# sara-nl/2D-VQ-AE-2

Measured on AMD Instinct MI355X. Metric: patches/sec (VQAE.forward: encoder -> VQ -> decoder), higher is better.
Workload: dtype f32; 1 GPU; BASELINE configs[1] (cfg B): batch 256/GPU of 256x256x3 fp32 -> 32x32 codes, K=256, D=128, full forward; global_batch=256, parallelism=patch-sharded x1

## Files before the change

### 2d-vq-ae-2_amd/csrc/conv_wino43.hip

```cpp
#include "kernels.h"
#include "mfma.h"

namespace {

using namespace vqae;

struct W43K {
    const float* __restrict__ t1;
    const float* __restrict__ U;
    const float* __restrict__ w3;
    const float* __restrict__ w1n;
    float* xio;
    float* y2;
    const float* __restrict__ Us;
    const float* __restrict__ w3s;
    const float* __restrict__ w1ns;
    int H, M;
    float act_a, act_b, t_scale, t_b4, n_b1a, n_b1b, n_b2a, n_b2b;
};

template <int C_, bool WIDE_ = false> struct W43Cfg {
    static constexpr int C = C_;
    static constexpr bool WIDE = WIDE_;
    static constexpr int BANDS = WIDE ? 2 : 1;
    static constexpr int ROWS = 8 * BANDS;
    static constexpr int W = C >= 128 ? 32 : 64;
    static constexpr int NT = (C == 256 || WIDE) ? 512 : 256;
    static constexpr int NWV = NT / 64;
    static constexpr int NS = C / 32;
    static constexpr int TG = NWV / NS;
    static constexpr int TILES = 16 * TG;
    static constexpr int TC = W / 4;
    static constexpr int PXH = 4 * W * BANDS;
    static constexpr int C4 = C / 4;
    static constexpr int RP = NT / C4;
    static constexpr int LDT = C + 4;
    static constexpr int KG = C / 16;
    static constexpr int KS = C / 8;
    static constexpr int NI = 2;
    static constexpr int WN = C / (32 * NI);
    static constexpr int MI = PXH / ((NWV / WN) * 32);
    static constexpr int V_BYTES = 6 * TILES * LDT * 4, T_BYTES = PXH * LDT * 4;
    static constexpr int LDS_BYTES = V_BYTES > T_BYTES ? V_BYTES : T_BYTES;
    static constexpr int LDVB = 3 * C + 8, KC = C / 32, KS2 = C / 16;
    static constexpr int VS_BYTES = 6 * TILES * LDVB * 2;
    static constexpr int LDS_SPLIT = VS_BYTES > T_BYTES ? VS_BYTES : T_BYTES;
    static_assert(TILES == 2 * TC * BANDS && RP == TC * BANDS && PXH / RP == 16 && MI * NI == 4, "geometry");
    static_assert(!WIDE || C == 128, "the wide form serves C = 128");
};
constexpr int EARLY = 1;
constexpr int RD = 4;
constexpr int NRES0 = 4;
constexpr int RT = 3;

__device__ __forceinline__ void split3(const f32x4& v, bf16x4 (&h)[3]) {
    h[0] = __builtin_convertvector(v, bf16x4);
    const f32x4 r1 = v - __builtin_convertvector(h[0], f32x4);
    h[1] = __builtin_convertvector(r1, bf16x4);
    const f32x4 r2 = r1 - __builtin_convertvector(h[1], f32x4);
    h[2] = __builtin_convertvector(r2, bf16x4);
}
__device__ __forceinline__ bf16x8 as_bf8(const f32x4& v) { return __builtin_bit_cast(bf16x8, v); }

__device__ __forceinline__ f32x4 fma4(const f32x4& a, float s, const f32x4& c) {
    return __builtin_elementwise_fma(a, f32x4{s, s, s, s}, c);
}

__device__ __forceinline__ f32x4 ldg(const float* sbase, unsigned voff_bytes) {
    return *reinterpret_cast<const f32x4*>(reinterpret_cast<const char*>(sbase) + voff_bytes);
}

template <int N> struct IC { static constexpr int value = N; };

constexpr int tail_row(int r) { return 8 * (r >> 2) + 4 * ((r >> 1) & 1) + (r & 1); }

template <int C, int TAIL, bool SPLIT, bool WIDE = false>
__global__ __launch_bounds__((W43Cfg<C, WIDE>::NT), (W43Cfg<C, WIDE>::NT == 512 ? 1 : 2))
void wino43_trunk_kernel(const W43K p) {
    using K = W43Cfg<C, WIDE>;
    static_assert(!WIDE || SPLIT, "the wide form is a split form");
    constexpr int W = K::W, LDT = K::LDT, KG = K::KG, KS = K::KS, TILES = K::TILES, TC = K::TC, NS = K::NS, C4 = K::C4, RP = K::RP;
    constexpr int MI = K::MI, NI = K::NI, WN = K::WN;
    constexpr int LDVB = K::LDVB, KC = K::KC, KS2 = K::KS2;
    extern __shared__ __attribute__((aligned(16))) float lds[];
    const int tid = threadIdx.x;
    const int lane = tid & 63;
    const int wave = __builtin_amdgcn_readfirstlane(tid >> 6);
    const int li = lane & 15, q = lane >> 4;
    const int ns = WIDE ? wave >> 1 : wave % NS, tg = WIDE ? 0 : wave / NS;

    int tile_m;
    {
        const int nwg = gridDim.x, bid = blockIdx.x;
        const int qq = nwg >> 3, r = nwg & 7, xcd = bid & 7;
        tile_m = (xcd < r ? xcd * (qq + 1) : r * (qq + 1) + (xcd - r) * qq) + (bid >> 3);
    }
    const int tpi = p.H / K::ROWS;
    const int img = tile_m / tpi;
    const int row0 = K::ROWS * (tile_m - img * tpi);
    const float* const xim = p.t1 + (int64_t)img * p.H * W * C;

    const int cg = tid % C4, tj = tid / C4;
    const int xcg = WIDE ? 8 * (wave & 3) + (lane & 7) : cg, tjc = WIDE ? lane >> 3 : tj, band = WIDE ? wave >> 2 : 0;
    constexpr int NCOL = WIDE ? 4 : 6, NB = NCOL / 2;
    unsigned coff[NCOL];
    int roff[2][6];
#pragma unroll
    for (int j = 0; j < NCOL; ++j) coff[j] = (unsigned)((((4 * tjc - 1 + j) & (W - 1)) * C + 4 * xcg) * 4);
#pragma unroll
    for (int s = 0; s < 2; ++s)
#pragma unroll
        for (int i = 0; i < 6; ++i) {
            int r = row0 + 8 * band + 4 * s - 1 + i;
            r = r < 0 ? r + p.H : (r >= p.H ? r - p.H : r);
            roff[s][i] = r * W * C;
        }

    f32x4 d[2][4][2];
    f32x4 w[6];
    auto issue = [&](auto kind_c, int k) __attribute__((always_inline)) {
        constexpr int KIND = decltype(kind_c)::value;
        const int s = k / NB, cp = k % NB, bf = k & 1;
#pragma unroll
        for (int i = 0; i < (KIND == 1 ? 4 : 3); ++i) {
            const int row = KIND == 0 ? 2 * i : (KIND == 5 ? 2 * i + 1 : i + 1);
#pragma unroll
            for (int jj = 0; jj < 2; ++jj) d[bf][i][jj] = ldg(xim + roff[s][row], coff[2 * cp + jj]);
        }
    };
    auto combine = [&](auto kind_c, int k, float c1, float c2, float c3) __attribute__((always_inline)) {
        constexpr int KIND = decltype(kind_c)::value;
        const int cp = k % NB, bf = k & 1;
#pragma unroll
        for (int jj = 0; jj < 2; ++jj) {
            if (KIND == 1) w[2 * cp + jj] = fma4(d[bf][0][jj], c1, fma4(d[bf][1][jj], c2, fma4(d[bf][2][jj], c3, d[bf][3][jj])));
            else w[2 * cp + jj] = fma4(d[bf][0][jj], 4.f, fma4(d[bf][1][jj], -5.f, d[bf][2][jj]));
        }
    };
    auto exchange = [&]() __attribute__((always_inline)) {
        const int nb = 4 * ((lane + 8) & 63);
#pragma unroll
        for (int jj = 0; jj < 2; ++jj)
#pragma unroll
            for (int e = 0; e < 4; ++e) {
                const float mine = w[jj][e];
                w[4 + jj][e] = __int_as_float(__builtin_amdgcn_ds_bpermute(nb, __float_as_int(mine)));
            }
    };
    auto columns = [&](int s) __attribute__((always_inline)) {
        const int slot = WIDE ? 4 * (tjc & 3) + 2 * (tjc >> 2) + s : s * TC + tjc;
        float* const dst = lds + (16 * band + slot) * LDT + 4 * xcg;
        __bf16* const dsb = reinterpret_cast<__bf16*>(lds) + (16 * band + slot) * LDVB + 4 * xcg;
        int vhi = 3 * TILES * LDVB;
        if constexpr (WIDE) asm volatile("" : "+v"(vhi));
        auto put = [&](int nu, const f32x4& v) __attribute__((always_inline)) {
            if constexpr (SPLIT) {
                bf16x4 h[3];
                split3(v, h);
#pragma unroll
                for (int pl = 0; pl < 3; ++pl) {
                    if (WIDE && nu >= 3) *reinterpret_cast<bf16x4*>(dsb + vhi + (nu - 3) * TILES * LDVB + pl * C) = h[pl];
                    else *reinterpret_cast<bf16x4*>(dsb + nu * TILES * LDVB + pl * C) = h[pl];
                }
            } else {
                *reinterpret_cast<f32x4*>(dst + nu * TILES * LDT) = v;
            }
        };
        const f32x4 t1 = fma4(w[2], -4.f, w[4]), t2 = fma4(w[1], -4.f, w[3]);
        const f32x4 t3 = w[4] - w[2], t4 = w[3] - w[1];
        put(0, fma4(w[0], 4.f, fma4(w[2], -5.f, w[4])));
        put(1, t1 + t2);
        put(2, t1 - t2);
        put(3, fma4(t4, 2.f, t3));
        put(4, fma4(t4, -2.f, t3));
        put(5, fma4(w[1], 4.f, fma4(w[3], -5.f, w[5])));
    };

    const float* const ub = p.U + ns * (KG * 512);
    const float* const ubs = p.Us + ns * (KC * 1536) + (WIDE ? 768 * (wave & 1) : 0);
    const __bf16* const vbs = reinterpret_cast<const __bf16*>(lds) + (16 * tg + li) * LDVB + 8 * q;
    const unsigned wl = 16u * lane;
    const float* const bfrag = lds + (16 * tg + li) * LDT + 4 * q;

    f32x4 Y[4][4][2];
#pragma unroll
    for (int a = 0; a < 4; ++a)
#pragma unroll
        for (int b = 0; b < 4; ++b) { Y[a][b][0] = f32x4{0.f, 0.f, 0.f, 0.f}; Y[a][b][1] = f32x4{0.f, 0.f, 0.f, 0.f}; }

    auto pass = [&](auto kind_c, auto next_c, int xi, float c1, float c2, float c3, float a1, float a2, float a3) __attribute__((always_inline)) {
        constexpr int KIND = decltype(kind_c)::value;
        constexpr int NEXT = decltype(next_c)::value;
        __builtin_amdgcn_sched_barrier(0);
#pragma unroll
        for (int j = 0; j < NCOL; ++j) asm volatile("" : "+v"(coff[j]));
        if (EARLY < 1) issue(kind_c, 0);
        if (EARLY < 2) issue(kind_c, 1);
#pragma unroll
        for (int k = 0; k < 2 * NB; ++k) {
            combine(kind_c, k, c1, c2, c3);
            if (k % NB == NB - 1) {
                if constexpr (WIDE) exchange();
                columns(k / NB);
            }
            if (k + 2 < 2 * NB) issue(kind_c, k + 2);
        }
        __builtin_amdgcn_sched_barrier(0);
        f32x4 Z[4][2];
        f32x4 acc[2][2];
        auto fold_nu = [&](int nu) __attribute__((always_inline)) {
#pragma unroll
            for (int bl = 0; bl < 2; ++bl) {
                if (nu == 0) Z[0][bl] = Z[0][bl] + acc[0][bl];
                if (nu == 2) {
                    const f32x4 sm = acc[1][bl] + acc[0][bl], df = acc[1][bl] - acc[0][bl];
                    Z[0][bl] = Z[0][bl] + sm; Z[2][bl] = Z[2][bl] + sm;
                    Z[1][bl] = Z[1][bl] + df; Z[3][bl] = Z[3][bl] + df;
                }
                if (nu == 4) {
                    const f32x4 sm = acc[1][bl] + acc[0][bl], df = acc[1][bl] - acc[0][bl];
                    Z[0][bl] = Z[0][bl] + sm; Z[2][bl] = fma4(sm, 4.f, Z[2][bl]);
                    Z[1][bl] = fma4(df, 2.f, Z[1][bl]); Z[3][bl] = fma4(df, 8.f, Z[3][bl]);
                }
                if (nu == 5) Z[3][bl] = Z[3][bl] + acc[1][bl];
            }
            if (nu == 0 || nu == 2 || nu == 4)
                asm volatile("" : "+v"(Z[0][0]), "+v"(Z[0][1]), "+v"(Z[1][0]), "+v"(Z[1][1]), "+v"(Z[2][0]), "+v"(Z[2][1]), "+v"(Z[3][0]), "+v"(Z[3][1]));
        };
        if constexpr (WIDE) {
            int64_t uoff = (int64_t)xi * 6 * (3 * C * C / 2);
            asm volatile("" : "+s"(uoff));
// ... 42 lines not shown
                    __builtin_amdgcn_sched_barrier(0);
                }
                fold_nu(nu);
            }
#undef WS
#undef VB
        } else if constexpr (SPLIT) {
            int64_t uoff = (int64_t)xi * 6 * (3 * C * C / 2);
            asm volatile("" : "+s"(uoff));
            const float* const ux = ubs + uoff;
#define WS(s, bl, pl) (((s) / KC) * (3 * C * C / 2) + 1536 * ((s) % KC) + 256 * (3 * (bl) + (pl)))
#define VB(s, pl) (*reinterpret_cast<const bf16x8*>(vbs + ((s) / KC) * TILES * LDVB + (pl) * C + 32 * ((s) % KC)))
            f32x4 w0[2][2], w1[2], w2[2];
#pragma unroll
            for (int bl = 0; bl < 2; ++bl) {
                w0[0][bl] = ldg(ux + WS(0, bl, 0), wl);
                w1[bl] = ldg(ux + WS(0, bl, 1), wl);
                w2[bl] = ldg(ux + WS(0, bl, 2), wl);
                w0[1][bl] = ldg(ux + WS(1, bl, 0), wl);
            }
            lds_barrier();
#pragma unroll
            for (int b = 0; b < 4; ++b) { Z[b][0] = f32x4{0.f, 0.f, 0.f, 0.f}; Z[b][1] = f32x4{0.f, 0.f, 0.f, 0.f}; }
            bf16x8 vb0 = VB(0, 0), vb1 = VB(0, 1), vb2 = VB(0, 2);
#pragma unroll
            for (int nu = 0; nu < 6; ++nu) {
                const int st = nu & 1;
                acc[st][0] = f32x4{0.f, 0.f, 0.f, 0.f};
                acc[st][1] = f32x4{0.f, 0.f, 0.f, 0.f};
#pragma unroll
                for (int kc = 0; kc < KC; ++kc) {
                    const int s = KC * nu + kc, sl = s & 1;
                    const bool nxt = s + 1 < 6 * KC;
#define MM(wa, vb) for (int bl = 0; bl < 2; ++bl) acc[st][bl] = __builtin_amdgcn_mfma_f32_16x16x32_bf16(as_bf8(wa[bl]), vb, acc[st][bl], 0, 0, 0)
                    MM(w1, vb1);
                    MM(w1, vb0);
                    if (nxt) for (int bl = 0; bl < 2; ++bl) w1[bl] = ldg(ux + WS(s + 1, bl, 1), wl);
                    MM(w2, vb0);
                    if (nxt) for (int bl = 0; bl < 2; ++bl) w2[bl] = ldg(ux + WS(s + 1, bl, 2), wl);
                    MM(w0[sl], vb2);
                    if (nxt) vb2 = VB(s + 1, 2);
                    MM(w0[sl], vb1);
                    if (nxt) vb1 = VB(s + 1, 1);
                    MM(w0[sl], vb0);
                    if (s + 2 < 6 * KC) for (int bl = 0; bl < 2; ++bl) w0[sl][bl] = ldg(ux + WS(s + 2, bl, 0), wl);
                    if (nxt) vb0 = VB(s + 1, 0);
#undef MM
                    __builtin_amdgcn_sched_barrier(0);
                }
                fold_nu(nu);
            }
#undef WS
#undef VB
        } else {
            int64_t uoff = (int64_t)xi * 6 * (C * C);
            asm volatile("" : "+s"(uoff));
            const float* const ux = ub + uoff;
#define WB(s) (((s) / KG) * (C * C) + 512 * ((s) % KG))
            f32x4 wq[RD][2];
#pragma unroll
            for (int s = 0; s < RD; ++s) {
                wq[s][0] = ldg(ux + WB(s), wl);
                wq[s][1] = ldg(ux + WB(s) + 256, wl);
            }
            lds_barrier();
#pragma unroll
            for (int b = 0; b < 4; ++b) { Z[b][0] = f32x4{0.f, 0.f, 0.f, 0.f}; Z[b][1] = f32x4{0.f, 0.f, 0.f, 0.f}; }
            f32x4 bq[2];
            bq[0] = *reinterpret_cast<const f32x4*>(bfrag);
#pragma unroll
            for (int nu = 0; nu < 6; ++nu) {
                const int st = nu & 1;
                acc[st][0] = f32x4{0.f, 0.f, 0.f, 0.f};
                acc[st][1] = f32x4{0.f, 0.f, 0.f, 0.f};
#pragma unroll
                for (int kg = 0; kg < KG; ++kg) {
                    const int s = KG * nu + kg;
                    if (s + 1 < 6 * KG)
                        bq[(s + 1) & 1] = *reinterpret_cast<const f32x4*>(bfrag + ((s + 1) / KG) * TILES * LDT + 16 * ((s + 1) % KG));
                    const f32x4 wa = wq[s % RD][0], wb = wq[s % RD][1];
                    if (s + RD < 6 * KG) {
                        wq[s % RD][0] = ldg(ux + WB(s + RD), wl);
                        wq[s % RD][1] = ldg(ux + WB(s + RD) + 256, wl);
                    }
#pragma unroll
                    for (int j = 0; j < 4; ++j) {
                        acc[st][0] = __builtin_amdgcn_mfma_f32_16x16x4f32(wa[j], bq[s & 1][j], acc[st][0], 0, 0, 0);
                        acc[st][1] = __builtin_amdgcn_mfma_f32_16x16x4f32(wb[j], bq[s & 1][j], acc[st][1], 0, 0, 0);
                    }
                    __builtin_amdgcn_sched_barrier(0);
                }
                fold_nu(nu);
            }
#undef WB
        }
        __builtin_amdgcn_sched_barrier(0);
        if constexpr (NEXT == 9) {
#pragma unroll
            for (int k = 0; k < EARLY; ++k)
#pragma unroll
                for (int i = 0; i < 4; ++i) {
                    const int ro = xi < 4 ? roff[0][i + 1] : roff[0][i < 3 ? 2 * i + 1 : 5];
#pragma unroll
                    for (int jj = 0; jj < 2; ++jj) d[k & 1][i][jj] = ldg(xim + ro, coff[2 * k + jj]);
                }
        } else {
// ... 111 lines not shown
                for (int mi = 0; mi < MI; ++mi) a[(ks + 1) & 1][mi] = *reinterpret_cast<const f32x4*>(a0 + mi * 32 * LDT + 8 * (ks + 1));
            }
            f32x4 bc[NI];
#pragma unroll
            for (int ni = 0; ni < NI; ++ni) bc[ni] = bt[ks % RT][ni];
            if (ks + RT < KS) {
#pragma unroll
                for (int ni = 0; ni < NI; ++ni) bt[ks % RT][ni] = ldg(b0 + ni * (KS * 256) + 256 * (ks + RT), wl);
            }
#pragma unroll
            for (int r = 0; r < 4; ++r)
#pragma unroll
                for (int mi = 0; mi < MI; ++mi)
#pragma unroll
                    for (int ni = 0; ni < NI; ++ni)
                        acc[mi][ni] = __builtin_amdgcn_mfma_f32_32x32x2f32(bc[ni][r], a[ks & 1][mi][r], acc[mi][ni], 0, 0, 0);
            __builtin_amdgcn_sched_barrier(0);
        }
    };
    auto acc_to_lds = [&]() __attribute__((always_inline)) {
#pragma unroll
        for (int ni = 0; ni < NI; ++ni)
#pragma unroll
            for (int mi = 0; mi < MI; ++mi)
#pragma unroll
                for (int g = 0; g < 4; ++g) {
                    f32x4 o;
#pragma unroll
                    for (int e = 0; e < 4; ++e) o[e] = acc[mi][ni][4 * g + e];
                    *reinterpret_cast<f32x4*>(T + (wm * MI * 32 + mi * 32 + li32) * LDT + (wn * NI + ni) * 32 + 8 * g + 4 * hh) = o;
                }
    };

#pragma unroll
    for (int hf = 0; hf < 2; ++hf) {
        int tbo = (2 * ty * W + 4 * tx) * LDT + 16 * wave + 4 * q, tro = tj0 * LDT + 4 * cg;
        if constexpr (WIDE) asm volatile("" : "+v"(tbo), "+v"(tro));
        int tbo1 = tbo + 4 * W * LDT, tro1 = tro + 8 * RP * LDT;
        if constexpr (WIDE) asm volatile("" : "+v"(tbo1), "+v"(tro1));
        auto tr = [&](int i) __attribute__((always_inline)) {
            if constexpr (WIDE) return reinterpret_cast<f32x4*>(T + (i < 8 ? tro + RP * i * LDT : tro1 + RP * (i - 8) * LDT));
            else return reinterpret_cast<f32x4*>(trow + RP * i * LDT);
        };
#pragma unroll
        for (int a2 = 0; a2 < 2; ++a2)
#pragma unroll
            for (int b = 0; b < 4; ++b)
#pragma unroll
                for (int bl = 0; bl < 2; ++bl) {
                    f32x4 o;
#pragma unroll
                    for (int e = 0; e < 4; ++e) o[e] = elu_act(Y[2 * hf + a2][b][bl][e] + p.act_a) + p.act_b;
                    if constexpr (WIDE) *reinterpret_cast<f32x4*>(T + (bl ? tbo1 : tbo) + (a2 * W + b) * LDT) = o;
                    else *reinterpret_cast<f32x4*>(T + ((2 * ty + a2) * W + 4 * tx + b) * LDT + 32 * ns + 16 * bl + 4 * q) = o;
                }
        tail_prefetch(SPLIT ? p.w3s : p.w3);
        [[maybe_unused]] float* xr[WIDE ? 1 : K::PXH / W];
        [[maybe_unused]] int64_t xu = 0;
        [[maybe_unused]] unsigned xvo = 0;
        if constexpr (WIDE) {
            xu = (((int64_t)img * p.H + row0 + 2 * hf) * W) * C;
            xvo = (unsigned)((tj0 * C + 4 * cg) * 4);
            asm volatile("" : "+v"(xvo));
        } else {
            const int64_t pixb = ((int64_t)img * p.H + row0 + 2 * hf) * W + tj0;
#pragma unroll
            for (int r = 0; r < K::PXH / W; ++r) xr[r] = p.xio + (pixb + (int64_t)(4 * (r >> 1) + (r & 1)) * W) * C + 4 * cg;
        }
        auto xp = [&](float* base, int i) __attribute__((always_inline)) {
            const int r = (RP * i) / W;
            if constexpr (WIDE) {
                int64_t ro = xu + (tail_row(r) * W + (RP * i) % W) * C;
                asm volatile("" : "+s"(ro));
                return reinterpret_cast<f32x4*>(reinterpret_cast<char*>(base + ro) + xvo);
            } else {
                return reinterpret_cast<f32x4*>(xr[r] + ((RP * i) % W) * C);
            }
        };
        f32x4 res[16];
#pragma unroll
        for (int i = 0; i < (hf == 0 ? NRES0 : 16); ++i) res[i] = __builtin_nontemporal_load(xp(p.xio, i));
        lds_barrier();
        gemm_tail(SPLIT ? p.w3s : p.w3);
        if (hf == 0) {
#pragma unroll
            for (int i = NRES0; i < 16; ++i) res[i] = __builtin_nontemporal_load(xp(p.xio, i));
        }
        if (TAIL == 2) tail_prefetch(SPLIT ? p.w1ns : p.w1n);
        lds_barrier();
        acc_to_lds();
        lds_barrier();
#pragma unroll
        for (int i = 0; i < 16; ++i) {
            f32x4 t = *tr(i);
            t = t * p.t_scale;
            t = t + p.t_b4;
            t = t + res[i];
            __builtin_nontemporal_store(t, xp(p.xio, i));
            if (TAIL == 2) {
#pragma unroll
                for (int e = 0; e < 4; ++e) t[e] = elu_act(t[e] + p.n_b1a) + p.n_b1b;
                *tr(i) = t;
            }
        }
        if constexpr (TAIL == 2) {
            lds_barrier();
// ... 60 lines not shown
        split3_f64(u[x], h);
        for (int pl = 0; pl < 3; ++pl) U[x * 3 * cc + fo + pl * 512] = h[pl];
    }
}

__global__ void split_1x1_kernel(const float* __restrict__ w, int c, __bf16* __restrict__ out) {
    const int i = blockIdx.x * blockDim.x + threadIdx.x;
    if (i >= c * c) return;
    const int n = i / c, k = i % c;
    __bf16 h[3];
    split3_f64((double)w[i], h);
    const int64_t fo = ((int64_t)(n >> 5) * (c / 16) + (k >> 4)) * 3 * 512 + (((k >> 3) & 1) * 32 + (n & 31)) * 8 + (k & 7);
    for (int pl = 0; pl < 3; ++pl) out[fo + pl * 512] = h[pl];
}

}

namespace vqae {

bool wino43_channels(int c) { return c == 256 || c == 128 || c == 64; }

bool wino43_supported(int c, int h, int w, int dtype) {
    return dtype == VQAE_DT_F32 && wino43_channels(c) && w == (c == 64 ? 64 : 32) && h >= 8 && h % 8 == 0;
}
bool wino43_enabled() { return env_int("VQAE_WINO43", 1) != 0; }

size_t wino43_weight_floats(int c) { return (size_t)36 * c * c; }

bool wino43_split_supported(int c) { return c == 128; }
size_t wino43_split_weight_bytes(int c) { return (size_t)36 * c * c * 3 * 2; }
size_t split_1x1_bytes(int c) { return (size_t)c * c * 3 * 2; }

int wino43_split_weight(const float* w_oihw_dev, int c, void* U_dev, hipStream_t stream) {
    VQAE_REQUIRE(wino43_split_supported(c), VQAE_ERR_UNSUPPORTED, "wino43_split_weight: C = %d", c);
    wino43_split_weight_kernel<<<(unsigned)ceil_div(c * c, 256), 256, 0, stream>>>(w_oihw_dev, c, (__bf16*)U_dev);
    VQAE_LAUNCH_CHECK();
    return VQAE_OK;
}

int split_1x1_weight(const float* w_packed_dev, int c, void* out_dev, hipStream_t stream) {
    VQAE_REQUIRE(wino43_split_supported(c), VQAE_ERR_UNSUPPORTED, "split_1x1_weight: C = %d", c);
    split_1x1_kernel<<<(unsigned)ceil_div(c * c, 256), 256, 0, stream>>>(w_packed_dev, c, (__bf16*)out_dev);
    VQAE_LAUNCH_CHECK();
    return VQAE_OK;
}

int wino43_transform_weight(const float* w_oihw_dev, int c, float* U_dev, hipStream_t stream) {
    VQAE_REQUIRE(wino43_channels(c), VQAE_ERR_UNSUPPORTED, "wino43_transform_weight: C = %d", c);
    wino43_weight_kernel<<<(unsigned)ceil_div(c * c, 256), 256, 0, stream>>>(w_oihw_dev, c, U_dev);
    VQAE_LAUNCH_CHECK();
    return VQAE_OK;
}

template <int C, bool SPLIT, bool WIDE = false>
static int launch_w43(W43K& k, int64_t M, bool chain, hipStream_t stream) {
    using K = W43Cfg<C, WIDE>;
    constexpr int lds = SPLIT ? K::LDS_SPLIT : K::LDS_BYTES;
    if (int rc = set_max_dynamic_lds((const void*)wino43_trunk_kernel<C, 1, SPLIT, WIDE>, lds)) return rc;
    if (int rc = set_max_dynamic_lds((const void*)wino43_trunk_kernel<C, 2, SPLIT, WIDE>, lds)) return rc;
    const unsigned grid = (unsigned)(M / (K::ROWS * K::W));
    const double flops = 2.0 * (double)M * C * (2.25 * C + C + (chain ? C : 0));
    ProfScope prof(C >= 128 ? PROF_CONV3X3_TRUNK : PROF_NONE, stream, flops);
    if (chain) wino43_trunk_kernel<C, 2, SPLIT, WIDE><<<grid, K::NT, lds, stream>>>(k);
    else wino43_trunk_kernel<C, 1, SPLIT, WIDE><<<grid, K::NT, lds, stream>>>(k);
    prof.done();
    VQAE_LAUNCH_CHECK();
    return VQAE_OK;
}

int wino43_trunk_tail(const float* t1, const float* U, const float* w3, float act_a, float act_b, float t_scale, float t_b4,
                      float* xio, const NextConv1& next, int batch, int h, int w, int c, hipStream_t stream,
                      const void* Us, const void* w3s) {
    if (batch == 0) return VQAE_OK;
    const float* w1n = (const float*)next.w1;
    float* t1_next = (float*)next.t1_next;
    VQAE_REQUIRE(t1 && U && w3 && xio && (!w1n || t1_next), VQAE_ERR_INVALID, "wino43_trunk_tail: null pointer");
    VQAE_REQUIRE(wino43_supported(c, h, w, VQAE_DT_F32), VQAE_ERR_UNSUPPORTED, "wino43_trunk_tail: C = %d, H = %d, W = %d", c, h, w);
    const int64_t M = (int64_t)batch * h * w;
    VQAE_REQUIRE(M < (1ll << 31) - 1024, VQAE_ERR_UNSUPPORTED, "wino43_trunk_tail: too many pixels");
    W43K k;
    memset(&k, 0, sizeof(k));
    k.t1 = t1; k.U = U; k.w3 = w3; k.w1n = w1n; k.xio = xio; k.y2 = t1_next;
    k.H = h; k.M = (int)M;
    k.act_a = act_a; k.act_b = act_b; k.t_scale = t_scale; k.t_b4 = t_b4;
    k.n_b1a = next.b1a; k.n_b1b = next.b1b; k.n_b2a = next.b2a; k.n_b2b = next.b2b;
    if (Us) {
        VQAE_REQUIRE(wino43_split_supported(c) && w3s && (!w1n || next.w1s), VQAE_ERR_INVALID, "wino43_trunk_tail: split form needs C = 128 and its three weights");
        k.Us = (const float*)Us; k.w3s = (const float*)w3s; k.w1ns = (const float*)next.w1s;
        if (h % 16 == 0) return launch_w43<128, true, true>(k, M, w1n != nullptr, stream);
        return launch_w43<128, true>(k, M, w1n != nullptr, stream);
    }
    switch (c) {
        case 256: return launch_w43<256, false>(k, M, w1n != nullptr, stream);
        case 128: return launch_w43<128, false>(k, M, w1n != nullptr, stream);
        default: return launch_w43<64, false>(k, M, w1n != nullptr, stream);
    }
}

}
```

### 2d-vq-ae-2_amd/csrc/handle.hip

```cpp
#include "kernels.h"

#include <algorithm>
#include <cmath>
#include <cstdlib>
#include <map>
#include <mutex>
#include <set>
#include <string>
#include <unordered_map>
#include <utility>
#include <vector>

namespace vqae {
char* last_error_buf() {
    static thread_local char buf[512] = {0};
    return buf;
}

ProfState& prof_state() {
    static ProfState p;
    return p;
}

int set_max_dynamic_lds(const void* kernel, int bytes) {
// ... 65 lines not shown
namespace {

enum { MODE_SAME = 0, MODE_DOWN = 1, MODE_UP = 2 };

struct Block : vqae::FixupScalars {
    int mode, cin, cout, br;
    float *w1, *w2, *w3, *wskip;
    float* wU43 = nullptr;
    void *wU43s = nullptr, *w1s = nullptr, *w3s = nullptr;
    float* wU = nullptr;
    float *w1f = nullptr, *w3f = nullptr;
    float *w2f = nullptr, *wskf = nullptr;
    void *w1h = nullptr, *w2h = nullptr, *w3h = nullptr, *wskh = nullptr;
    int kind = VQAE_BLOCK_FIXUP, hidden = 0;
    float *bv1 = nullptr, *bv2 = nullptr, *bv3 = nullptr;
    float *fc0w = nullptr, *fc0b = nullptr, *fc2w = nullptr, *fc2b = nullptr;
};

const float kMean255[3] = {0.7279f * 255.0f, 0.5955f * 255.0f, 0.7762f * 255.0f};
const float kInv255[3] = {1.0f / (0.2419f * 255.0f), 1.0f / (0.3083f * 255.0f), 1.0f / (0.1741f * 255.0f)};
const float kStd255[3] = {0.2419f * 255.0f, 0.3083f * 255.0f, 0.1741f * 255.0f};

}

struct vqae_handle {
    vqae_config cfg;
    int C = 0, D = 0, K = 0;
    std::vector<Block> enc, dec;
    float *stem_w = nullptr, *stem_b = nullptr, *ostem_w = nullptr, *ostem_b = nullptr;
    void *stem_wh = nullptr, *ostem_wh = nullptr;
    bool fuse_stem16 = true;
    float *embed = nullptr;
    float *pin_w = nullptr, *pin_b = nullptr, *pout_w = nullptr, *pout_b = nullptr;
    float *pin_wt = nullptr, *pout_wr = nullptr;
    bool fuse_vq = true;
    std::vector<void*> owned;
    float* buf[4] = {nullptr, nullptr, nullptr, nullptr};
    size_t buf_floats = 0;
    void* vq_ws = nullptr;
    size_t vq_ws_bytes = 0;
    float* loss_scratch = nullptr;
    int device = 0;
    bool has_encoder = false, has_decoder = false;
    bool fuse_trunk = true;
    bool t1_ready = false;
    bool up_conv_first = true;
    bool fuse_down = true;
    bool fuse_down16 = true;
    bool fuse_up16 = true;
    bool fuse_up_tail = true;
    bool fuse_up_head = true;
    bool use_wino = true;
    bool w43_split = true;
    void* idx_scratch = nullptr;
    size_t idx_scratch_bytes = 0;
    float* se_ws = nullptr;
    size_t se_ws_bytes = 0;
    size_t se_gate_off = 0;
};

namespace {

using TensorMap = std::unordered_map<std::string, const vqae_tensor*>;

int find(const TensorMap& tm, const std::string& name, int64_t numel, const float** out) {
    auto it = tm.find(name);
    if (it == tm.end()) return vqae::fail(VQAE_ERR_NOT_FOUND, "missing tensor '%s'", name.c_str());
    if (it->second->numel != numel)
        return vqae::fail(VQAE_ERR_INVALID, "tensor '%s' has %lld elements, expected %lld", name.c_str(),
                          (long long)it->second->numel, (long long)numel);
    *out = it->second->data;
    return VQAE_OK;
}

int dev_alloc(vqae_handle* h, size_t bytes, void** out) {
    void* p = nullptr;
    if (hipMalloc(&p, bytes ? bytes : 16) != hipSuccess)
        return vqae::fail(VQAE_ERR_NOMEM, "hipMalloc of %zu bytes failed", bytes);
    h->owned.push_back(p);
    *out = p;
    return VQAE_OK;
}

int upload(vqae_handle* h, const float* host, int64_t numel, float** out) {
    void* p;
    int rc = dev_alloc(h, (size_t)numel * 4, &p);
    if (rc) return rc;
    VQAE_HIP_CHECK(hipMemcpy(p, host, (size_t)numel * 4, hipMemcpyHostToDevice));
    *out = (float*)p;
    return VQAE_OK;
}

template <class Transform>
int upload_via(vqae_handle* h, const float* host, size_t in_bytes, size_t out_bytes, const char* what, Transform transform, void** out) {
    void* tmp = nullptr;
    if (hipMalloc(&tmp, in_bytes) != hipSuccess) return vqae::fail(VQAE_ERR_NOMEM, "hipMalloc failed");
    const hipError_t e = hipMemcpy(tmp, host, in_bytes, hipMemcpyHostToDevice);
    void* dst = nullptr;
    int rc = (e == hipSuccess) ? dev_alloc(h, out_bytes, &dst) : vqae::fail(VQAE_ERR_HIP, "hipMemcpy failed: %s", hipGetErrorString(e));
    if (rc == VQAE_OK) rc = transform((const float*)tmp, dst);
    if (rc == VQAE_OK && hipDeviceSynchronize() != hipSuccess) rc = vqae::fail(VQAE_ERR_HIP, "%s failed", what);
    (void)hipFree(tmp);
    *out = dst;
    return rc;
}

// ... 272 lines not shown
    if (b.mode == MODE_SAME) {
        if (b.w2h && h->fuse_trunk && vqae::same16_16_supported(b.cin, H, W, dt)) return R_SAME16_16;
        if (b.w2h && h->fuse_trunk && vqae::trunk16_supported(b.cin, H, W, dt)) return R_TRUNK16;
        if (b.wU && h->fuse_trunk && vqae::wino_trunk_supported(b.cin, H, W, dt)) {
            if (!(b.wU43 && vqae::wino43_supported(b.cin, H, W, dt))) return R_WINO;
            const bool chain = same_width_next(b, next) && next->w1f;
            return b.wU43s && (!chain || next->w1s) ? R_WINO43_SPLIT : R_WINO43;
        }
        if (vqae::conv_trunk_tail_channels(b.cin) && b.cout == b.cin && h->fuse_trunk) return R_TAIL;
        if (b.w2h && !f32 && vqae::same8_16_supported(b.cin, H, W, dt)) return R_SAME8_16;
        if (b.cin == b.cout && vqae_fixup_same_supported(b.cin, H, W)) return R_FIXUP_FUSED;
        return R_SAME;
    }
    if (b.mode == MODE_DOWN) {
        if (b.w2h && !f32 && vqae::down16_supported(b.cin, H, W)) return R_DOWN16;
        if (b.w2f && vqae::down_block_supported(b.cin, H, W)) return R_DOWN_FUSED;
        return R_DOWN;
    }
    if (f32 && h->up_conv_first) return h->fuse_up_tail && vqae::up_tail_supported(b.br, b.cout) ? R_UP_CONV_FIRST_TAIL : R_UP_CONV_FIRST;
    if (b.w2h && vqae::up16_supported(b.cin, H, W, dt) && vqae::trunk16_head_supported(b.cin, (int64_t)B * H * W, dt)) return R_UP16;
    return R_UP;
}

int run_conv1(const vqae_handle* h, const Block& b, int B, int H, int W, const float* x, float* y, hipStream_t st) {
    return conv(ConvCall(h, B, H, W, b.cin, b.br, 1, 1, 0, VQAE_PAD_NONE).pre(VQAE_PRE_BIAS_ELU_BIAS, b.b1a, b.b1b).act(b.b2a, b.b2b), x, b.w1, nullptr, y, st);
}

int run_trunk(vqae_handle* h, Route r, const Block& b, const Block* next, int B, int H, int W, hipStream_t st) {
    float *X = h->buf[0], *P = h->buf[1], *Q = h->buf[2];
    const int dt = h->cfg.compute_dtype;
    const int64_t M = (int64_t)B * H * W;
    const bool t16 = r == R_TRUNK16, wino = r == R_WINO43_SPLIT || r == R_WINO43 || r == R_WINO;
    int rc;
    if (!h->t1_ready) {
        if (t16 && vqae::trunk16_head_supported(b.cin, M, dt)) {
            rc = vqae::trunk16_head(X, b.w1h, b.b1a, b.b1b, b.b2a, b.b2b, P, M, b.cin, dt, false, st);
        } else if (t16) {
            if ((rc = run_conv1(h, b, B, H, W, X, Q, st))) return rc;
            rc = vqae::trunk16_round_pack(Q, P, M * b.cin, dt, st);
        } else if (wino && dt == VQAE_DT_F32 && vqae::fixup_conv1_supported(b.cin, M)) {
            rc = vqae::fixup_conv1(X, b.w1f, b.b1a, b.b1b, b.b2a, b.b2b, P, M, b.cin, st);
        } else {
            rc = run_conv1(h, b, B, H, W, X, P, st);
        }
        if (rc) return rc;
    }
    vqae::NextConv1 nx;
    const void* next_w1 = !same_width_next(b, next) ? nullptr : (t16 ? next->w1h : (const void*)next->w1f);
    if (next_w1) nx = {next_w1, next->w1s, next->b1a, next->b1b, next->b2a, next->b2b, Q};
    if (t16) {
        rc = vqae::trunk16_block(P, b.w2h, b.w3h, b.b3a, b.b3b, b.scale, b.b4, X, nx, B, H, W, b.cin, dt, st);
    } else if (r == R_WINO43_SPLIT || r == R_WINO43) {
        rc = vqae::wino43_trunk_tail(P, b.wU43, b.w3f, b.b3a, b.b3b, b.scale, b.b4, X, nx, B, H, W, b.cin, st,
                                     r == R_WINO43_SPLIT ? b.wU43s : nullptr, b.w3s);
    } else if (r == R_WINO) {
        rc = vqae::wino_trunk_tail(P, b.wU, b.w3f, b.b3a, b.b3b, b.scale, b.b4, X, nx, B, H, W, b.cin, dt, st);
    } else {
        const ConvCall c2 = ConvCall(h, B, H, W, b.br, b.br, 3, 1, 1, VQAE_PAD_CIRCULAR).act(b.b3a, b.b3b);
        rc = vqae::conv_trunk_tail(&c2.a, P, b.w2, b.w3f, b.scale, b.b4, X, nx, st);
    }
    if (rc) return rc;
    if (nx.w1) std::swap(h->buf[1], h->buf[2]);
    h->t1_ready = nx.w1 != nullptr;
    return VQAE_OK;
}

int run_block(vqae_handle* h, const Block& b, const Block* next, int B, int& H, int& W, hipStream_t st) {
    if (b.kind == VQAE_BLOCK_MBCONV) return run_mbconv(h, b, B, H, W, st);
    float *X = h->buf[0], *P = h->buf[1], *Q = h->buf[2], *R = h->buf[3];
    const int dt = h->cfg.compute_dtype;
    const Route r = select_route(h, b, next, B, H, W);
    if (r >= R_TRUNK16 && r <= R_TAIL) return run_trunk(h, r, b, next, B, H, W, st);
    h->t1_ready = false;
    int rc;
    float* out = X;
    switch (r) {
    case R_SAME16_16:
        if ((rc = vqae::same16_16_block(X, P, b.w1h, b.w2h, b.w3h, B, H, W, b.cin, b, dt, st))) return rc;
        out = P;
        break;
    case R_SAME8_16:
        if ((rc = vqae::same8_16_block(X, P, b.w1, b.w2h, b.w3h, B, H, W, b, dt, st))) return rc;
        out = P;
        break;
    case R_FIXUP_FUSED:
        if ((rc = vqae_fixup_same_block_f32(X, P, b.w1, b.w2, b.w3, B, H, W, b.cin, &b.b1a, dt, st))) return rc;
        out = P;
        break;
    case R_SAME:
        if ((rc = run_conv1(h, b, B, H, W, X, P, st))) return rc;
        if ((rc = conv(ConvCall(h, B, H, W, b.br, b.br, 3, 1, 1, VQAE_PAD_CIRCULAR).act(b.b3a, b.b3b), P, b.w2, nullptr, Q, st))) return rc;
        if ((rc = conv(ConvCall(h, B, H, W, b.br, b.cout, 1, 1, 0, VQAE_PAD_NONE).scale_bias(b.scale, b.b4), Q, b.w3, X, X, st))) return rc;
        break;
    case R_DOWN16:
        if ((rc = vqae::down16_block(X, b.w1h, b.w2h, b.w3h, b.wskh, B, H, W, b.cin, b, dt, R, st))) return rc;
        out = R;
        break;
    case R_DOWN_FUSED:
        if ((rc = vqae::down_block(X, b.w1f, b.w2f, b.w3f, b.wskf, B, H, W, b.cin, b, dt, R, st))) return rc;
        out = R;
        break;
    case R_DOWN:
        if ((rc = conv(ConvCall(h, B, H, W, b.cin, b.cout, 2, 2, 0, VQAE_PAD_NONE).pre(VQAE_PRE_BIAS, b.b1c, 0.f).bias(b.b1d), X, b.wskip, nullptr, R, st))) return rc;
        if ((rc = run_conv1(h, b, B, H, W, X, P, st))) return rc;
        if ((rc = conv(ConvCall(h, B, H, W, b.br, b.br, 2, 2, 0, VQAE_PAD_NONE).act(b.b3a, b.b3b), P, b.w2, nullptr, Q, st))) return rc;
        if ((rc = conv(ConvCall(h, B, H / 2, W / 2, b.br, b.cout, 1, 1, 0, VQAE_PAD_NONE).scale_bias(b.scale, b.b4), Q, b.w3, R, R, st))) return rc;
        out = R;
// ... 154 lines not shown

int run_decoder_convs(vqae_handle* h, int B, int qh, int qw, int layout, float* out, hipStream_t st) {
    const int dt = h->cfg.compute_dtype;
    int H = qh, W = qw, rc;
    h->t1_ready = false;
    for (size_t i = 0; i < h->dec.size(); ++i)
        if ((rc = run_block(h, h->dec[i], i + 1 < h->dec.size() ? &h->dec[i + 1] : nullptr, B, H, W, st))) return rc;
    if (!out) out = h->buf[1];
    if (h->ostem_wh && vqae::stem16_supported(h->cfg.stem, H, W, dt))
        return vqae::ostem16(h->buf[0], h->ostem_wh, h->ostem_b, B, H, W, h->cfg.stem, out, layout == VQAE_LAYOUT_NCHW ? 1 : 0, dt, st);
    return vqae::conv3x3_direct(h->buf[0], 0, nullptr, nullptr, h->ostem_w, h->ostem_b, B, H, W, h->cfg.stem,
                                h->cfg.in_channels, out, layout == VQAE_LAYOUT_NCHW ? 1 : 0, dt, st);
}

int export_q(vqae_handle* h, int B, int zh, int zw, int layout, float* q, hipStream_t st) {
    if (!q) return VQAE_OK;
    if (layout == VQAE_LAYOUT_NCHW) return vqae_nhwc_to_nchw_f32(h->buf[0], B, h->C, zh, zw, q, st);
    VQAE_HIP_CHECK(hipMemcpyAsync(q, h->buf[0], (size_t)B * zh * zw * h->C * 4, hipMemcpyDeviceToDevice, st));
    return VQAE_OK;
}

}

extern "C" int vqae_create(const vqae_config* cfg, const vqae_tensor* tensors, int n_tensors, vqae_handle** out) {
    VQAE_REQUIRE(cfg && tensors && out, VQAE_ERR_INVALID, "vqae_create: null pointer");
    VQAE_REQUIRE(cfg->in_channels == 3, VQAE_ERR_UNSUPPORTED, "in_channels %d (only 3)", cfg->in_channels);
    VQAE_REQUIRE(cfg->stem >= 4 && cfg->stem % 4 == 0 && cfg->stem <= 64, VQAE_ERR_UNSUPPORTED, "stem %d", cfg->stem);
    VQAE_REQUIRE(cfg->stem % 8 == 0, VQAE_ERR_UNSUPPORTED, "stem %d must be a multiple of 8", cfg->stem);
    VQAE_REQUIRE(cfg->n_down >= 1 && cfg->n_down <= 6 && cfg->n_pre >= 0 && cfg->n_post >= 0 && cfg->n_enc >= 0,
                 VQAE_ERR_INVALID, "bad depth parameters");
    VQAE_REQUIRE(cfg->num_embeddings >= 1 && cfg->num_embeddings <= 65536, VQAE_ERR_UNSUPPORTED, "num_embeddings %d",
                 cfg->num_embeddings);
    VQAE_REQUIRE(cfg->projection_dim == 0 || (cfg->projection_dim % 8 == 0), VQAE_ERR_UNSUPPORTED,
                 "projection_dim %d must be 0 or a multiple of 8", cfg->projection_dim);
    VQAE_REQUIRE(cfg->compute_dtype >= VQAE_DT_F32 && cfg->compute_dtype <= VQAE_DT_F16, VQAE_ERR_INVALID,
                 "compute_dtype %d", cfg->compute_dtype);
    VQAE_REQUIRE(cfg->block_kind == VQAE_BLOCK_FIXUP || cfg->block_kind == VQAE_BLOCK_MBCONV, VQAE_ERR_INVALID,
                 "block_kind %d", cfg->block_kind);
    if (cfg->block_kind == VQAE_BLOCK_MBCONV) {
        VQAE_REQUIRE(cfg->compute_dtype == VQAE_DT_F32, VQAE_ERR_UNSUPPORTED, "MBConv blocks run in fp32 only");
        VQAE_REQUIRE(cfg->expand_ratio >= 1 && cfg->se_divisor >= 1 && cfg->bn_eps > 0.f, VQAE_ERR_INVALID,
                     "MBConv: expand_ratio %d, se_divisor %d, bn_eps %g", cfg->expand_ratio, cfg->se_divisor, (double)cfg->bn_eps);
    }
    TensorMap tm;
    for (int i = 0; i < n_tensors; ++i) tm[tensors[i].name] = &tensors[i];

    vqae_handle* h = new vqae_handle();
    h->cfg = *cfg;
    if (hipGetDevice(&h->device) != hipSuccess) { delete h; return vqae::fail(VQAE_ERR_HIP, "hipGetDevice failed"); }
    h->fuse_trunk = vqae::env_int("VQAE_NO_TRUNK_FUSION", 0) == 0;
    h->up_conv_first = vqae::env_int("VQAE_NO_UP_REORDER", 0) == 0;
    h->use_wino = vqae::env_int("VQAE_NO_WINOGRAD", 0) == 0;
    h->w43_split = vqae::env_int("VQAE_W43_SPLIT", 1) != 0;
    h->fuse_up_tail = vqae::env_int("VQAE_NO_UP_TAIL_FUSION", 0) == 0;
    h->fuse_up_head = vqae::env_int("VQAE_NO_UP_HEAD_FUSION", 0) == 0;
    h->fuse_down = vqae::env_int("VQAE_NO_DOWN_FUSION", 0) == 0;
    h->fuse_down16 = vqae::env_int("VQAE_NO_DOWN16", 0) == 0;
    h->fuse_up16 = vqae::env_int("VQAE_NO_UP16", 0) == 0;
    h->fuse_stem16 = vqae::env_int("VQAE_NO_STEM16", 0) == 0;
    h->fuse_vq = vqae::env_int("VQAE_NO_VQ_FUSION", 0) == 0;
    h->C = cfg->stem << cfg->n_down;
    h->D = cfg->projection_dim > 0 ? cfg->projection_dim : h->C;
    h->K = cfg->num_embeddings;
    int rc = VQAE_OK;
    const float* p;
    auto bail = [&](int code) { vqae_destroy(h); return code; };

    const bool has_enc = tm.count("encoder.in_stem.weight") > 0;
    const bool has_dec = tm.count("decoder.out_stem.weight") > 0;
    if (!has_enc && !has_dec) return bail(vqae::fail(VQAE_ERR_NOT_FOUND, "neither encoder.* nor decoder.* tensors given"));
    h->has_encoder = has_enc;
    h->has_decoder = has_dec;
    int c = cfg->stem << cfg->n_down;
    const std::string vq = "encoder.vq_layers.0.";

    const bool stem16 = cfg->compute_dtype != VQAE_DT_F32 && h->fuse_stem16 && cfg->in_channels == 3 && vqae::stem16_channels(cfg->stem);
    auto pack_stem16 = [&](const float* w, int n_out, int cin, void** dst) {
        if (int r = dev_alloc(h, vqae::stem16_weight_bytes(cin), dst)) return r;
        return vqae::stem16_pack_weight(w, n_out, cin, cfg->compute_dtype, *dst, nullptr);
    };
    if (has_enc) {
        if ((rc = find(tm, "encoder.in_stem.weight", (int64_t)cfg->stem * 3 * 9, &p)) || (rc = upload(h, p, (int64_t)cfg->stem * 27, &h->stem_w))) return bail(rc);
        if ((rc = find(tm, "encoder.in_stem.bias", cfg->stem, &p)) || (rc = upload(h, p, cfg->stem, &h->stem_b))) return bail(rc);
        if (stem16 && (rc = pack_stem16(h->stem_w, cfg->stem, 3, &h->stem_wh))) return bail(rc);
        c = cfg->stem;
        if ((rc = load_levels(h, tm, "encoder.down_layers.0.layers.", MODE_DOWN, &c, &h->enc))) return bail(rc);
        if ((rc = load_same_run(h, tm, "encoder.pre_enc_layers.0.", 0, cfg->n_enc, c, &h->enc))) return bail(rc);
    }
    if (has_enc || tm.count(vq + "embed")) {
        if ((rc = find(tm, vq + "embed", (int64_t)h->K * h->D, &p)) || (rc = upload(h, p, (int64_t)h->K * h->D, &h->embed))) return bail(rc);
        if (cfg->projection_dim > 0) {
            if ((rc = find(tm, vq + "proj_in.weight", (int64_t)h->D * h->C, &p)) || (rc = upload_packed(h, p, h->D, h->C, 1, &h->pin_w))) return bail(rc);
            if ((rc = find(tm, vq + "proj_in.bias", h->D, &p)) || (rc = upload(h, p, h->D, &h->pin_b))) return bail(rc);
            if ((rc = vqae_round_inplace_f32(h->pin_b, h->D, cfg->compute_dtype, nullptr))) return bail(rc);
            if ((rc = find(tm, vq + "proj_out.weight", (int64_t)h->C * h->D, &p)) || (rc = upload_packed(h, p, h->C, h->D, 1, &h->pout_w))) return bail(rc);
            if ((rc = find(tm, vq + "proj_out.bias", h->C, &p)) || (rc = upload(h, p, h->C, &h->pout_b))) return bail(rc);
            if ((rc = vqae_round_inplace_f32(h->pout_b, h->C, cfg->compute_dtype, nullptr))) return bail(rc);
            if (h->D == 8) {
                std::vector<float> wt((size_t)h->C * 8);
                const float* pi = tm.at(vq + "proj_in.weight")->data;
                for (int j = 0; j < 8; ++j) for (int cc = 0; cc < h->C; ++cc) wt[(size_t)cc * 8 + j] = pi[(size_t)j * h->C + cc];
                if ((rc = upload(h, wt.data(), (int64_t)h->C * 8, &h->pin_wt)) ||
                    (rc = upload(h, tm.at(vq + "proj_out.weight")->data, (int64_t)h->C * 8, &h->pout_wr))) return bail(rc);
                if ((rc = vqae_round_inplace_f32(h->pin_wt, (int64_t)h->C * 8, cfg->compute_dtype, nullptr)) ||
                    (rc = vqae_round_inplace_f32(h->pout_wr, (int64_t)h->C * 8, cfg->compute_dtype, nullptr))) return bail(rc);
            }
// ... 293 lines not shown
```

### 2d-vq-ae-2_amd/csrc/kernels.h

```cpp
#pragma once
#include "common.h"

namespace vqae {

struct FixupScalars {
    float b1a, b1b, b2a, b2b, b3a, b3b, b4, scale, b1c, b1d;
};
static_assert(sizeof(FixupScalars) == 10 * sizeof(float), "FixupScalars is read as float[8] / float[10]");

struct NextConv1 {
    const void* w1 = nullptr;
    const void* w1s = nullptr;
    float b1a = 0.f, b1b = 0.f, b2a = 0.f, b2b = 0.f;
    void* t1_next = nullptr;
};

bool conv_trunk_tail_channels(int c);
int conv_tail_kslice(int dtype, int cin);
int conv_trunk_tail(const vqae_conv_args* a, const float* t1, const float* w2, const float* w3, float t_scale, float t_b4,
                    float* xio, const NextConv1& next, hipStream_t stream);

bool wino_trunk_channels(int c, int dtype);
bool wino_trunk_supported(int c, int h, int w, int dtype);
size_t wino_weight_floats(int c);
int wino_transform_weight(const float* w_oihw_dev, int c, int dtype, float* U_dev, hipStream_t stream);
int frag_weight(const float* w_packed_dev, int n_rows, int K, int sk, float* out_dev, hipStream_t stream);
int wino_trunk_tail(const float* t1, const float* U, const float* w3, float act_a, float act_b, float t_scale, float t_b4,
                    float* xio, const NextConv1& next, int batch, int h, int w, int c, int dtype, hipStream_t stream);
bool fixup_conv1_supported(int c, int64_t m);
int fixup_conv1(const float* x, const float* w1f, float pa, float pb, float aa, float ab, float* y, int64_t m, int c,
                hipStream_t stream);

bool wino43_channels(int c);
bool wino43_supported(int c, int h, int w, int dtype);
bool wino43_enabled();
size_t wino43_weight_floats(int c);
int wino43_transform_weight(const float* w_oihw_dev, int c, float* U_dev, hipStream_t stream);
bool wino43_split_supported(int c);
size_t wino43_split_weight_bytes(int c);
size_t split_1x1_bytes(int c);
int wino43_split_weight(const float* w_oihw_dev, int c, void* U_dev, hipStream_t stream);
int split_1x1_weight(const float* w_packed_dev, int c, void* out_dev, hipStream_t stream);
int wino43_trunk_tail(const float* t1, const float* U, const float* w3, float act_a, float act_b, float t_scale, float t_b4,
                      float* xio, const NextConv1& next, int batch, int h, int w, int c, hipStream_t stream,
                      const void* Us, const void* w3s);

bool trunk16_channels(int c);
bool trunk16_supported(int c, int h, int w, int dtype);
size_t trunk16_weight_bytes(int c, int taps);
int trunk16_round_pack(const float* src, void* dst, int64_t n, int dtype, hipStream_t stream);
bool trunk16_head_supported(int c, int64_t m, int dtype);
int trunk16_head(const float* x, const void* w1f, float b1a, float b1b, float b2a, float b2b, void* t1, int64_t m, int c,
                 int dtype, bool out32, hipStream_t stream);
int trunk16_block(const void* t1, const void* w2f, const void* w3f, float act_a, float act_b, float t_scale, float t_b4,
                  float* xio, const NextConv1& next, int batch, int h, int w, int c, int dtype, hipStream_t stream);

bool same8_16_channels(int c);
bool same8_16_supported(int c, int h, int w, int dtype);
int same8_16_block(const float* x, float* y, const float* w1_packed, const void* w2h, const void* w3h, int B, int H, int W,
                   const FixupScalars& s, int dtype, hipStream_t stream);
bool same16_16_supported(int c, int h, int w, int dtype);
int same16_16_block(const float* x, float* y, const void* w1h, const void* w2h, const void* w3h, int B, int H, int W, int c,
                    const FixupScalars& s, int dtype, hipStream_t stream);

bool down_block_channels(int cin);
bool down_block_supported(int cin, int h, int w);
int down_block(const float* x, const float* w1f, const float* w2f, const float* w3f, const float* wskf, int B, int H, int W,
               int cin, const FixupScalars& s, int dtype, float* y, hipStream_t stream);
bool down16_channels(int cin);
bool down16_supported(int cin, int h, int w);
size_t down16_weight_bytes(int n_rows, int K);
int pack16_weight(const float* w_packed_dev, int n_rows, int K, int dtype, void* out_dev, hipStream_t stream);
int down16_block(const float* x, const void* w1h, const void* w2h, const void* w3h, const void* wskh, int B, int H, int W,
                 int cin, const FixupScalars& s, int dtype, float* y, hipStream_t stream);

bool up16_channels(int c);
bool up16_supported(int c, int h, int w, int dtype);
int up16_block(const float* x, const float* t1, const void* w2h, const void* w3h, const void* wskh, int B, int H, int W, int c,
               const FixupScalars& s, int dtype, float* y, hipStream_t stream);

bool stem16_channels(int c0);
bool stem16_supported(int c0, int h, int w, int dtype);
size_t stem16_weight_bytes(int cin);
int stem16_pack_weight(const float* w_dev, int n_out, int cin, int dtype, void* out_dev, hipStream_t stream);
int istem16(const void* x, int x_kind, const float* mean255, const float* inv_std255, const void* wf, const float* bias, int B,
            int H, int W, int c0, float* y, int dtype, hipStream_t stream);
int ostem16(const float* x, const void* wf, const float* bias, int B, int H, int W, int c, float* y, int y_nchw, int dtype,
            hipStream_t stream);

bool up_head_channels(int c);
int up_head(const float* x, const float* w1f, const float* w2f, const float* wskf, int64_t M, int c, const FixupScalars& s,
            float* q, float* r, hipStream_t stream);
bool up_tail_supported(int cb, int co);
int up_tail(const float* q, const float* s, const float* w3_packed, int B, int H, int W, int cb, int co, float b3a, float b3b,
            float scale, float b4, float* y, hipStream_t stream);

bool conv_small_k_supported(const vqae_conv_args* a);
int conv_small_k(const vqae_conv_args* a, const float* x, const float* w, const float* bias_vec, const float* residual,
// ... 36 lines not shown
```

Before: 4621 patches/s.

## Add shared-tile wave mapping for C=64 fp32 Winograd trunk kernel

Adds a SHARED variant of the Winograd F(4,3) trunk kernel for C=64 fp32. Each pair of waves splits the output channels and shares the same tile rows, so B fragments from LDS are reused across two n-halves per wave. It also deepens the weight register prefetch ring to six stages and remaps the epilogue write into the T buffer. The variant is on by default and can be turned off with an environment flag; the trade is a different register and LDS access pattern.

```diff
diff --git a/2d-vq-ae-2_amd/csrc/conv_wino43.hip b/2d-vq-ae-2_amd/csrc/conv_wino43.hip
--- a/2d-vq-ae-2_amd/csrc/conv_wino43.hip
+++ b/2d-vq-ae-2_amd/csrc/conv_wino43.hip
@@ -50,6 +50,7 @@
 };
 constexpr int EARLY = 1;
 constexpr int RD = 4;
+constexpr int RDS = 6;
 constexpr int NRES0 = 4;
 constexpr int RT = 3;
 
@@ -74,11 +75,12 @@
 
 constexpr int tail_row(int r) { return 8 * (r >> 2) + 4 * ((r >> 1) & 1) + (r & 1); }
 
-template <int C, int TAIL, bool SPLIT, bool WIDE = false>
+template <int C, int TAIL, bool SPLIT, bool WIDE = false, bool SHARED = false>
 __global__ __launch_bounds__((W43Cfg<C, WIDE>::NT), (W43Cfg<C, WIDE>::NT == 512 ? 1 : 2))
 void wino43_trunk_kernel(const W43K p) {
     using K = W43Cfg<C, WIDE>;
     static_assert(!WIDE || SPLIT, "the wide form is a split form");
+    static_assert(!SHARED || (C == 64 && !SPLIT && !WIDE), "the shared form serves the fp32 kernel at C = 64");
     constexpr int W = K::W, LDT = K::LDT, KG = K::KG, KS = K::KS, TILES = K::TILES, TC = K::TC, NS = K::NS, C4 = K::C4, RP = K::RP;
     constexpr int MI = K::MI, NI = K::NI, WN = K::WN;
     constexpr int LDVB = K::LDVB, KC = K::KC, KS2 = K::KS2;
@@ -87,7 +89,7 @@
     const int lane = tid & 63;
     const int wave = __builtin_amdgcn_readfirstlane(tid >> 6);
     const int li = lane & 15, q = lane >> 4;
-    const int ns = WIDE ? wave >> 1 : wave % NS, tg = WIDE ? 0 : wave / NS;
+    const int ns = WIDE || SHARED ? wave >> 1 : wave % NS, tg = WIDE || SHARED ? 0 : wave / NS;
 
     int tile_m;
     {
@@ -176,7 +178,7 @@
         put(5, fma4(w[1], 4.f, fma4(w[3], -5.f, w[5])));
     };
 
-    const float* const ub = p.U + ns * (KG * 512);
+    const float* const ub = p.U + ns * (KG * 512) + (SHARED ? 256 * (wave & 1) : 0);
     const float* const ubs = p.Us + ns * (KC * 1536) + (WIDE ? 768 * (wave & 1) : 0);
     const __bf16* const vbs = reinterpret_cast<const __bf16*>(lds) + (16 * tg + li) * LDVB + 8 * q;
     const unsigned wl = 16u * lane;
@@ -325,6 +327,46 @@
             }
 #undef WS
 #undef VB
+        } else if constexpr (SHARED) {
+            int64_t uoff = (int64_t)xi * 6 * (C * C);
+            asm volatile("" : "+s"(uoff));
+            const float* const ux = ub + uoff;
+#define WB(s) (((s) / KG) * (C * C) + 512 * ((s) % KG))
+#define VF(s, g) (*reinterpret_cast<const f32x4*>(bfrag + (g) * 16 * LDT + ((s) / KG) * TILES * LDT + 16 * ((s) % KG)))
+            f32x4 wq[RDS];
+#pragma unroll
+            for (int s = 0; s < RDS; ++s) wq[s] = ldg(ux + WB(s), wl);
+            lds_barrier();
+#pragma unroll
+            for (int b = 0; b < 4; ++b) { Z[b][0] = f32x4{0.f, 0.f, 0.f, 0.f}; Z[b][1] = f32x4{0.f, 0.f, 0.f, 0.f}; }
+            f32x4 bq[2][2];
+            bq[0][0] = VF(0, 0);
+            bq[0][1] = VF(0, 1);
+#pragma unroll
+            for (int nu = 0; nu < 6; ++nu) {
+                const int st = nu & 1;
+                acc[st][0] = f32x4{0.f, 0.f, 0.f, 0.f};
+                acc[st][1] = f32x4{0.f, 0.f, 0.f, 0.f};
+#pragma unroll
+                for (int kg = 0; kg < KG; ++kg) {
+                    const int s = KG * nu + kg;
+                    if (s + 1 < 6 * KG) {
+                        bq[(s + 1) & 1][0] = VF(s + 1, 0);
+                        bq[(s + 1) & 1][1] = VF(s + 1, 1);
+                    }
+                    const f32x4 wa = wq[s % RDS];
+                    if (s + RDS < 6 * KG) wq[s % RDS] = ldg(ux + WB(s + RDS), wl);
+#pragma unroll
+                    for (int j = 0; j < 4; ++j) {
+                        acc[st][0] = __builtin_amdgcn_mfma_f32_16x16x4f32(wa[j], bq[s & 1][0][j], acc[st][0], 0, 0, 0);
+                        acc[st][1] = __builtin_amdgcn_mfma_f32_16x16x4f32(wa[j], bq[s & 1][1][j], acc[st][1], 0, 0, 0);
+                    }
+                    __builtin_amdgcn_sched_barrier(0);
+                }
+                fold_nu(nu);
+            }
+#undef WB
+#undef VF
         } else {
             int64_t uoff = (int64_t)xi * 6 * (C * C);
             asm volatile("" : "+s"(uoff));
@@ -542,6 +584,7 @@
 #pragma unroll
                     for (int e = 0; e < 4; ++e) o[e] = elu_act(Y[2 * hf + a2][b][bl][e] + p.act_a) + p.act_b;
                     if constexpr (WIDE) *reinterpret_cast<f32x4*>(T + (bl ? tbo1 : tbo) + (a2 * W + b) * LDT) = o;
+                    else if constexpr (SHARED) *reinterpret_cast<f32x4*>(T + ((2 * bl + a2) * W + 4 * li + b) * LDT + 16 * wave + 4 * q) = o;
                     else *reinterpret_cast<f32x4*>(T + ((2 * ty + a2) * W + 4 * tx + b) * LDT + 32 * ns + 16 * bl + 4 * q) = o;
                 }
         tail_prefetch(SPLIT ? p.w3s : p.w3);
@@ -708,17 +751,17 @@
     return VQAE_OK;
 }
 
-template <int C, bool SPLIT, bool WIDE = false>
+template <int C, bool SPLIT, bool WIDE = false, bool SHARED = false>
 static int launch_w43(W43K& k, int64_t M, bool chain, hipStream_t stream) {
     using K = W43Cfg<C, WIDE>;
     constexpr int lds = SPLIT ? K::LDS_SPLIT : K::LDS_BYTES;
-    if (int rc = set_max_dynamic_lds((const void*)wino43_trunk_kernel<C, 1, SPLIT, WIDE>, lds)) return rc;
-    if (int rc = set_max_dynamic_lds((const void*)wino43_trunk_kernel<C, 2, SPLIT, WIDE>, lds)) return rc;
+    if (int rc = set_max_dynamic_lds((const void*)wino43_trunk_kernel<C, 1, SPLIT, WIDE, SHARED>, lds)) return rc;
+    if (int rc = set_max_dynamic_lds((const void*)wino43_trunk_kernel<C, 2, SPLIT, WIDE, SHARED>, lds)) return rc;
     const unsigned grid = (unsigned)(M / (K::ROWS * K::W));
     const double flops = 2.0 * (double)M * C * (2.25 * C + C + (chain ? C : 0));
     ProfScope prof(C >= 128 ? PROF_CONV3X3_TRUNK : PROF_NONE, stream, flops);
-    if (chain) wino43_trunk_kernel<C, 2, SPLIT, WIDE><<<grid, K::NT, lds, stream>>>(k);
-    else wino43_trunk_kernel<C, 1, SPLIT, WIDE><<<grid, K::NT, lds, stream>>>(k);
+    if (chain) wino43_trunk_kernel<C, 2, SPLIT, WIDE, SHARED><<<grid, K::NT, lds, stream>>>(k);
+    else wino43_trunk_kernel<C, 1, SPLIT, WIDE, SHARED><<<grid, K::NT, lds, stream>>>(k);
     prof.done();
     VQAE_LAUNCH_CHECK();
     return VQAE_OK;
@@ -726,7 +769,7 @@
 
 int wino43_trunk_tail(const float* t1, const float* U, const float* w3, float act_a, float act_b, float t_scale, float t_b4,
                       float* xio, const NextConv1& next, int batch, int h, int w, int c, hipStream_t stream,
-                      const void* Us, const void* w3s) {
+                      const void* Us, const void* w3s, bool c64_shared) {
     if (batch == 0) return VQAE_OK;
     const float* w1n = (const float*)next.w1;
     float* t1_next = (float*)next.t1_next;
@@ -749,7 +792,9 @@
     switch (c) {
         case 256: return launch_w43<256, false>(k, M, w1n != nullptr, stream);
         case 128: return launch_w43<128, false>(k, M, w1n != nullptr, stream);
-        default: return launch_w43<64, false>(k, M, w1n != nullptr, stream);
+        default:
+            if (c64_shared) return launch_w43<64, false, false, true>(k, M, w1n != nullptr, stream);
+            return launch_w43<64, false>(k, M, w1n != nullptr, stream);
     }
 }
 
diff --git a/2d-vq-ae-2_amd/csrc/handle.hip b/2d-vq-ae-2_amd/csrc/handle.hip
--- a/2d-vq-ae-2_amd/csrc/handle.hip
+++ b/2d-vq-ae-2_amd/csrc/handle.hip
@@ -141,6 +141,7 @@
     bool fuse_up_head = true;
     bool use_wino = true;
     bool w43_split = true;
+    bool w43_c64_shared = true;
     void* idx_scratch = nullptr;
     size_t idx_scratch_bytes = 0;
     float* se_ws = nullptr;
@@ -519,7 +520,7 @@
         rc = vqae::trunk16_block(P, b.w2h, b.w3h, b.b3a, b.b3b, b.scale, b.b4, X, nx, B, H, W, b.cin, dt, st);
     } else if (r == R_WINO43_SPLIT || r == R_WINO43) {
         rc = vqae::wino43_trunk_tail(P, b.wU43, b.w3f, b.b3a, b.b3b, b.scale, b.b4, X, nx, B, H, W, b.cin, st,
-                                     r == R_WINO43_SPLIT ? b.wU43s : nullptr, b.w3s);
+                                     r == R_WINO43_SPLIT ? b.wU43s : nullptr, b.w3s, h->w43_c64_shared);
     } else if (r == R_WINO) {
         rc = vqae::wino_trunk_tail(P, b.wU, b.w3f, b.b3a, b.b3b, b.scale, b.b4, X, nx, B, H, W, b.cin, dt, st);
     } else {
@@ -780,6 +781,7 @@
     h->up_conv_first = vqae::env_int("VQAE_NO_UP_REORDER", 0) == 0;
     h->use_wino = vqae::env_int("VQAE_NO_WINOGRAD", 0) == 0;
     h->w43_split = vqae::env_int("VQAE_W43_SPLIT", 1) != 0;
+    h->w43_c64_shared = vqae::env_int("VQAE_W43_C64_SHARED", 1) != 0;
     h->fuse_up_tail = vqae::env_int("VQAE_NO_UP_TAIL_FUSION", 0) == 0;
     h->fuse_up_head = vqae::env_int("VQAE_NO_UP_HEAD_FUSION", 0) == 0;
     h->fuse_down = vqae::env_int("VQAE_NO_DOWN_FUSION", 0) == 0;
diff --git a/2d-vq-ae-2_amd/csrc/kernels.h b/2d-vq-ae-2_amd/csrc/kernels.h
--- a/2d-vq-ae-2_amd/csrc/kernels.h
+++ b/2d-vq-ae-2_amd/csrc/kernels.h
@@ -43,7 +43,7 @@
 int split_1x1_weight(const float* w_packed_dev, int c, void* out_dev, hipStream_t stream);
 int wino43_trunk_tail(const float* t1, const float* U, const float* w3, float act_a, float act_b, float t_scale, float t_b4,
                       float* xio, const NextConv1& next, int batch, int h, int w, int c, hipStream_t stream,
-                      const void* Us, const void* w3s);
+                      const void* Us, const void* w3s, bool c64_shared);
 
 bool trunk16_channels(int c);
 bool trunk16_supported(int c, int h, int w, int dtype);
```

Result: no change. 4632 patches/s (median of 6 runs) (+0.2%).
